# fzi-forschungszentrum-informatik/muvo

Measured on AMD Instinct MI355X. Metric: world-model training samples/sec (seq_len=10), higher is better.
Workload: dtype f32 storage/accumulate; large contractions (convolutions, transformer Linear) as bf16x3 split products

## Files before the change

### include/muvo_hip.h

```cpp
#ifndef MUVO_HIP_H
#define MUVO_HIP_H
#include <stdint.h>

#ifdef __cplusplus
extern "C" {
#endif

#define MUVO_OK 0
#define MUVO_ERR_INVALID_ARG (-1)
#define MUVO_ERR_HIP (-2)

#define MUVO_ACT_NONE 0
#define MUVO_ACT_RELU 1
#define MUVO_ACT_LEAKY 2
#define MUVO_ACT_ELU 3
#define MUVO_ACT_TANH 4
#define MUVO_ACT_SIGMOID 5

const char* muvo_last_error(void);
int muvo_abi_version(void);
int muvo_selftest_mfma(void* stream);
int muvo_set_deterministic(int on);
int muvo_reset_accumulators(void);
int muvo_get_deterministic(void);
// ... 5 lines not shown
  int32_t in_sz[3], out_sz[3];
  int32_t ksz[3], stride[3], pad[3], dil[3];
} muvo_conv_desc;

#define MUVO_CONV_F32 0
#define MUVO_CONV_BF16X3 1
#define MUVO_CONV_MODE_DEFAULT MUVO_CONV_BF16X3
int muvo_conv_set_products(int n);
int muvo_conv_get_products(void);
int muvo_conv_set_mode(int mode);
int muvo_conv_get_mode(void);
int muvo_conv_set_bf16x3_min_gflop(double gflop_per_item);
int muvo_linear_bf16x3_pack_floats(int in_f, int out_f, int64_t* fwd_floats, int64_t* dgrad_floats);
int muvo_linear_bf16x3_pack(int in_f, int out_f, const float* w, float* wp_fwd, float* wp_dgrad, void* stream);
int64_t muvo_linear_bf16x3_workspace_bytes(int64_t rows, int features);
int muvo_linear_bf16x3_split(const float* x, int64_t rows, int features, void* ws, void* stream);
int muvo_linear_bf16x3_forward(int64_t rows, int in_f, int out_f, const void* ws_x, const float* wp_fwd, const float* bias,
                               float* y, int act, float slope, void* stream);
int muvo_linear_bf16x3_dgrad(int64_t rows, int in_f, int out_f, const void* ws_dz, const float* wp_dgrad, float* dx,
                             void* stream);
int muvo_linear_bf16x3_wgrad(int64_t rows, int in_f, int out_f, const void* ws_x, const void* ws_dz, float* scratch,
                             float* dw, void* stream);
int64_t muvo_pack_table_item_bytes(void);
int muvo_conv_pack_table_add(void* host_items, int capacity, int* n_items, int64_t* n_blocks, const muvo_conv_desc* d,
                             const float* w, float* wp_fwd, float* wp_dgrad);
int muvo_linear_bf16x3_pack_table_add(void* host_items, int capacity, int* n_items, int64_t* n_blocks, int in_f, int out_f,
                                      const float* w, float* wp_fwd, float* wp_dgrad);
int muvo_pack_table_run(const void* dev_items, int n_items, int64_t n_blocks, void* stream);
int muvo_conv_pack_sizes(const muvo_conv_desc* d, int64_t* fwd_floats, int64_t* dgrad_floats);
int muvo_conv_pack_weights(const muvo_conv_desc* d, const float* w, float* wp_fwd, float* wp_dgrad, void* stream);
int64_t muvo_conv_workspace_bytes(const muvo_conv_desc* d, int op);
int muvo_conv_kernel_family(const muvo_conv_desc* d, int op);
int muvo_conv_kernel_variant(const muvo_conv_desc* d, int op);
int muvo_conv_forward(const muvo_conv_desc* d, const float* x, const float* wp_fwd, const float* bias, float* y, int act,
                      float slope, void* ws, void* stream);
int muvo_conv_dgrad(const muvo_conv_desc* d, const float* dy, const float* wp_dgrad, float* dx, void* ws, int ws_valid,
                    void* stream);
int muvo_conv_forward_head_supported(const muvo_conv_desc* d, int CO);
int muvo_conv_forward_head(const muvo_conv_desc* d, const float* x, const float* wp_fwd, const float* bias, float* y, int act,
                           float slope, void* ws, const float* head_w, const float* head_b, int CO, float* logits, void* stream);
int muvo_conv_forward_moments_supported(const muvo_conv_desc* d);
int muvo_conv_forward_moments(const muvo_conv_desc* d, const float* x, const float* wp_fwd, const float* bias, float* y, int act,
                              float slope, double* moments, void* stream);
int muvo_adain_fwd_moments(const float* x, const float* style, float* y, float* save_mean, float* save_rstd, double* moments,
                           int N, int C, int64_t S, float eps, void* stream);
int muvo_adain_affine(const float* style, double* moments, float* save_mean, float* save_rstd, float* aff, int N, int C, int64_t S,
                      float eps, void* stream);
int muvo_conv_affine_supported(const muvo_conv_desc* d);
int muvo_conv_forward_affine(const muvo_conv_desc* d, const float* x, const float* aff, const float* wp_fwd, const float* bias,
                             float* y, int act, float slope, double* moments, void* stream);
int muvo_conv_wgrad_affine(const muvo_conv_desc* d, const float* x, const float* aff, const float* dy, float* dw, float* dbias,
                           void* stream);
int muvo_grouped_linear_fwd(const float* x, int M, int K, int L, const float* const* W, const float* const* b, float* const* Y,
                            const int* N, void* stream);
int muvo_grouped_linear_bwd(const float* x, int M, int K, int L, const float* const* W, float* const* dY, float* dx,
                            float* const* dW, float* const* db, const int* N, void* stream);
int muvo_bf3_loop_clock(double* shader_mhz, double* us_per_k_step);
int muvo_adain_head_supported(int C, int CO, int64_t S);
int muvo_adain_head_fwd(const float* x, const float* style, float* save_mean, float* save_rstd, double* moments, const float* head_w,
                        const float* head_b, float* logits, int N, int C, int CO, int64_t S, float eps, void* stream);
int muvo_adain_head_bwd(const float* x, const float* style, const float* save_mean, const float* save_rstd, const float* head_w,
                        const float* dlogits, float* dx, float* dstyle, float* dhead_w, float* dhead_b, double* ws, int N, int C,
                        int CO, int64_t S, int act, float slope, void* stream);
int muvo_conv_dgrad_accumulate(const muvo_conv_desc* d, const float* dy, const float* wp_dgrad, float* dx, void* stream);
int muvo_conv_prepare_dy(const muvo_conv_desc* d, const float* y, const float* dy, int act, float slope, void* ws_dy,
                         float* dbias, void* stream);
// ... 210 lines not shown
```

### muvo_amd/csrc/conv_bf3.h

```cpp
#pragma once
#include "conv_plan.h"

void bf3_finish_phase(ConvPhase& g);
int bf3_pack_phase(const ConvPhase& g, const float* w, float* wp, hipStream_t st);
long bf3_workspace_bytes(int N, int C, long S);
int bf3_split_input(const float* x, void* ws, int N, int C, long S, hipStream_t st, const float* yact = nullptr, int act = 0,
                    float slope = 0.f, float* dbias = nullptr, const float* dhead = nullptr, const float* head_w = nullptr, int CO = 0,
                    float* dhead_w = nullptr, float* dhead_b = nullptr);
int bf3_launch_fwd_phase(const ConvPhase& g, const void* ws, const float* wp, const float* bias, float* out, int act,
                         float slope, hipStream_t st, int ksplit = 1);
void bf3_set_fused_head(const float* w, const float* b, float* out, int co);
void bf3_set_products(int n);
int bf3_get_products();
int bf3_fwd_ksplit(const ConvPhase& g);
int bf3_wgrad_phase(const ConvPhase& g, const void* ws_x, int Cin_total, const void* ws_dz, int Cout_total, float* wg,
                    float* dw, hipStream_t st);
int bf3_split_rows(const float* x, void* ws, long rows, int C, hipStream_t st);
bool bf3_fwd_uses_pp(const ConvPhase& g);
bool bf3_wgrad_uses_pp(const ConvPhase& g);
struct PackItem {
  ConvPhase g;
  const float* w;
  float* dst;
  long blk0;
  int nblk, pad_;
};
int pack_table_launch(const PackItem* dev_items, int n, long n_blocks, hipStream_t st);
```

### muvo_amd/csrc/conv_bf3.hip

```cpp
#include "conv_bf3.h"
#include <type_traits>

typedef __bf16 bf16x8 __attribute__((ext_vector_type(8)));
typedef __bf16 bf16x2 __attribute__((ext_vector_type(2)));
typedef float f32x2 __attribute__((ext_vector_type(2)));

__device__ unsigned long long g_bf3_clock[3];
extern "C" int muvo_bf3_loop_clock(double* shader_mhz, double* us_per_k_step) {
  unsigned long long h[3] = {0, 0, 0};
  if (hipMemcpyFromSymbol(h, HIP_SYMBOL(g_bf3_clock), sizeof(h)) != hipSuccess) return MUVO_ERR_HIP;
  if (h[1] == 0 || h[2] == 0) { *shader_mhz = 0.0; *us_per_k_step = 0.0; return MUVO_OK; }
  *shader_mhz = (double)h[0] / ((double)h[1] / 100.0);
  *us_per_k_step = (double)h[1] / 100.0 / (double)h[2];
  return MUVO_OK;
}

#ifdef MUVO_BF3_STAMPS
__device__ unsigned long long g_bf3_stamps[8 * 16384];
#define BF3_STAMP(slot)                                                                      \
  if (MUVO_BF3_STAMPS != 3 && threadIdx.x == 0 && blockIdx.x < 16384) g_bf3_stamps[blockIdx.x * 8 + (slot)] = __builtin_amdgcn_s_memrealtime()
extern "C" int muvo_debug_bf3_stamps_reset() {
  void* p = nullptr;
  return hipGetSymbolAddress(&p, HIP_SYMBOL(g_bf3_stamps)) == hipSuccess && hipMemset(p, 0, sizeof(unsigned long long) * 8 * 16384) == hipSuccess ? 0 : 1;
}
extern "C" int muvo_debug_bf3_stamps(unsigned long long* host_out, int n_u64) {
  return hipMemcpyFromSymbol(host_out, HIP_SYMBOL(g_bf3_stamps), sizeof(unsigned long long) * n_u64) == hipSuccess ? 0 : 1;
}
#define BF3_LINEAR_BLOCK ((blockIdx.z * gridDim.y + blockIdx.y) * gridDim.x + blockIdx.x)
#define BF3_STAMP3(slot)                                                                     \
  if (threadIdx.x == 0 && BF3_LINEAR_BLOCK < 16384) g_bf3_stamps[BF3_LINEAR_BLOCK * 8 + (slot)] = __builtin_amdgcn_s_memrealtime()
#else
#define BF3_STAMP(slot)
#define BF3_STAMP3(slot)
#endif

__device__ __forceinline__ void split2(float x0, float x1, unsigned& hi, unsigned& lo) {
  const bf16x2 h = __builtin_convertvector((f32x2){x0, x1}, bf16x2);
  hi = __builtin_bit_cast(unsigned, h);
  const float h0 = __uint_as_float(hi << 16), h1 = __uint_as_float(hi & 0xffff0000u);
  const bf16x2 l = __builtin_convertvector((f32x2){x0 - h0, x1 - h1}, bf16x2);
  lo = __builtin_bit_cast(unsigned, l);
}


typedef const __attribute__((address_space(1))) void* gptr_t;
typedef __attribute__((address_space(3))) void* lptr_t;
__host__ __device__ static inline bool bf3_tap_inner(const ConvPhase& g) { return (g.Cp & 31) == 0 && g.T > 1; }

__device__ __forceinline__ void dma16(const uint4* g, uint4* lds_wave_base) {
  __builtin_amdgcn_global_load_lds((gptr_t)g, (lptr_t)lds_wave_base, 16, 0, 0);
}

template <int BM, int BN, int WM, int WN, int BKC, int NST, bool ONE = false>
__global__ void __launch_bounds__(64 * WM * WN)
conv_bf3_kernel(const ConvPhase g, const uint4* __restrict__ xs, long plane_u4, const uint4* __restrict__ wp,
                const float* __restrict__ bias, float* __restrict__ out, int act, float slope,
                const uint4* __restrict__ zero16, int ksplit, const float* __restrict__ head_w, const float* __restrict__ head_b,
                float* __restrict__ head_out, int head_co) {
  constexpr int BK = 8 * BKC, NW = WM * WN;
  constexpr int TM = BM / (WM * 32), TN = BN / (WN * 32);
  constexpr int STAGE = 2 * BKC * (BM + BN);
  constexpr int RG = BM / 64, NG = BN / 64;
  constexpr int APW = 2 * BKC * RG / NW;
  constexpr int CPW = 2 * BKC * NG / NW;
  static_assert(APW * NW == 2 * BKC * RG && CPW * NW == 2 * BKC * NG && NW % NG == 0, "DMA roles must tile");
  constexpr int DMA_PER_STEP = APW + CPW;
  extern __shared__ uint4 smem[];
  const int tid = threadIdx.x, lane = tid & 63;
  const int wave = __builtin_amdgcn_readfirstlane(tid >> 6);
  const int wm = wave / WN, wn = wave % WN;
  BF3_STAMP(0);
#if defined(MUVO_BF3_STAMPS) && MUVO_BF3_STAMPS != 3
  if (threadIdx.x == 0 && blockIdx.x < 16384)
    g_bf3_stamps[blockIdx.x * 8 + 5] = ((unsigned long long)__builtin_amdgcn_s_getreg(63508) << 32) | __builtin_amdgcn_s_getreg(63492);
#endif

  const int gx = (g.npix + BN - 1) / BN;
  const int wg = xcd_swizzle(blockIdx.x, gridDim.x);
  const int bx = wg % gx, by = wg / gx;

  constexpr int NPS = CPW / 2;
  static_assert(CPW % 2 == 0 && NPS * NW * 16 == BN, "B load roles must tile");
  const int cp8 = g.Cp >> 3;
  int* taptab = (int*)(smem + NST * STAGE);
  for (int tt = tid; tt < g.T; tt += 64 * NW) {
    const int d = g.tap_d[tt];
    taptab[tt] = (((((d >> 16) & 255) - 128) * g.IH + ((d >> 8) & 255) - 128) * g.IW + (d & 255) - 128) * cp8;
    taptab[64 + tt] = d;
  }
  float* head_lds = (float*)(taptab + 128) + NW * (32 * TM);
  if (head_co > 0)
    for (int i = tid; i < head_co * g.Msub; i += 64 * NW) head_lds[i] = head_w[i];
  __syncthreads();
  int pixoff[NPS];
  unsigned long long vmask[NPS];
  int z0[NPS], y0[NPS], x0[NPS];
  bool pvalid[NPS];
#pragma unroll
  for (int sidx = 0; sidx < NPS; ++sidx) {
    const int p = bx * BN + (wave * NPS + sidx) * 16 + (lane >> 2);
    pvalid[sidx] = p < g.npix;
    int n, iz, iy, ix;
    decode_pix(g, pvalid[sidx] ? p : 0, n, iz, iy, ix);
    z0[sidx] = iz * g.is[0] + g.ib[0]; y0[sidx] = iy * g.is[1] + g.ib[1]; x0[sidx] = ix * g.is[2] + g.ib[2];
    pixoff[sidx] = (((n * g.ID + z0[sidx]) * g.IH + y0[sidx]) * g.IW + x0[sidx]) * cp8;
    vmask[sidx] = 0ull;
  }
#pragma unroll 3
  for (int tt = 0; tt < g.T; ++tt) {
    const int d = taptab[64 + tt];
    const int dz = ((d >> 16) & 255) - 128, dy = ((d >> 8) & 255) - 128, dx = (d & 255) - 128;
#pragma unroll
    for (int sidx = 0; sidx < NPS; ++sidx) {
      const bool ok = pvalid[sidx] && (unsigned)(z0[sidx] + dz) < (unsigned)g.ID && (unsigned)(y0[sidx] + dy) < (unsigned)g.IH &&
                      (unsigned)(x0[sidx] + dx) < (unsigned)g.IW;
      vmask[sidx] |= (unsigned long long)ok << tt;
    }
  }
  const int zero_off = (int)(2 * plane_u4);
  const int m_tile = by * BM;
  const uint4* wpb = wp + g.wp_off / 4 + m_tile;
  const int nk = g.Kp / BK;
  const int sps = (nk + ksplit - 1) / ksplit;
  const int kt0 = blockIdx.y * sps, kt1 = kt0 + sps < nk ? kt0 + sps : nk;
  if (kt0 >= kt1) return;

  float* sbias = (float*)(taptab + 128) + wave * (32 * TM);
  typedef unsigned u32x4 __attribute__((ext_vector_type(4)));
  const __amdgpu_buffer_rsrc_t rs_w = __builtin_amdgcn_make_buffer_rsrc(
      (void*)wpb, 0, (int)(((long)(g.Kp >> 5) * 8 * g.Mp - m_tile) * 16), 0x00020000);
  const __amdgpu_buffer_rsrc_t rs_x = __builtin_amdgcn_make_buffer_rsrc((void*)xs, 0, (int)(2 * plane_u4 * 16), 0x00020000);
  constexpr int OOB = 0x7ffffff0;
  u32x4 R[2][DMA_PER_STEP];
  int b_uoff = 0; unsigned long long b_bit = 0ull; bool b_tval = false;
  const bool tap_inner = bf3_tap_inner(g);
  int ti_t = kt0 % g.T, ti_c8 = (lane & 3) + 4 * (kt0 / g.T);
  auto bstate = [&](int kt) {
    if (tap_inner) {
      b_uoff = taptab[ti_t] + ti_c8;
      b_bit = 1ull << ti_t;
      b_tval = ti_c8 < cp8;
      if (++ti_t == g.T) { ti_t = 0; ti_c8 += 4; }
      return;
    }
    const int k0 = kt * BK + (lane & 3) * 8;
    const int t = (int)(((unsigned long long)(unsigned)k0 * g.cp_magic) >> 32);
    const int c8 = (k0 - t * g.Cp) >> 3;
    const int tc = t < g.T ? t : 0;
    b_uoff = taptab[tc] + c8;
    b_bit = 1ull << tc;
    b_tval = t < g.T;
  };
  auto gload_piece = [&](auto par, int kt, int q) {
    constexpr int P = decltype(par)::value;
    if (q < APW) {
      const int k32 = (kt * BK) >> 5, c4 = ((kt * BK) >> 3) & 3;
      const int a = wave * APW + q;
      const int pc = a / RG, rg = a % RG;
      const int plane = pc / BKC, ch = pc % BKC;
      R[P][q] = __builtin_bit_cast(u32x4, __builtin_amdgcn_raw_buffer_load_b128(rs_w, (ONE && plane == 1) ? OOB : lane * 16, ((k32 * 8 + plane * 4 + c4 + ch) * g.Mp + rg * 64) * 16, 0));
    } else {
      const int plane = (q - APW) & 1, sidx = (q - APW) >> 1;
      const bool ok = b_tval && (vmask[sidx] & b_bit) && !(ONE && plane == 1);
      const int off = ok ? (pixoff[sidx] + b_uoff + plane * (int)plane_u4) * 16 : OOB;
      R[P][q] = __builtin_bit_cast(u32x4, __builtin_amdgcn_raw_buffer_load_b128(rs_x, off, 0, 0));
    }
  };
  auto lstore_piece = [&](auto par, int stage, int q) {
    constexpr int P = decltype(par)::value;
    uint4* S = smem + stage * STAGE;
    if (q < APW) {
      const int a = wave * APW + q;
      const int pc = a / RG, rg = a % RG;
      *(u32x4*)(S + pc * BM + rg * 64 + lane) = R[P][q];
    } else {
      const int pl = (wave * NPS + ((q - APW) >> 1)) * 16 + (lane >> 2);
      *(u32x4*)(S + 2 * BKC * BM + ((q - APW) & 1) * BKC * BN + pl * 4 + ((lane & 3) ^ ((lane >> 4) & 3))) = R[P][q];
    }
  };

  f32x16 acc[TM][TN];
#pragma unroll
  for (int i = 0; i < TM; ++i)
#pragma unroll
    for (int j = 0; j < TN; ++j)
#pragma unroll
      for (int r = 0; r < 16; ++r) acc[i][j][r] = 0.f;

  static_assert(BKC == 4 && (NST == 2 || NST == 3), "two k-slices per step; two LDS stages, or three for the ping-pong schedule");
  const int fragA = wm * (TM * 32) + (lane & 31);
  const int fragB = 2 * BKC * BM + (wn * (TN * 32) + (lane & 31)) * 4 + ((lane >> 5) ^ ((lane >> 2) & 3));
  auto load_frags = [&](int stage, int ks, bf16x8 (&ah)[TM], bf16x8 (&al)[TM], bf16x8 (&bh)[TN], bf16x8 (&bl)[TN]) {
    const uint4* S = smem + stage * STAGE;
// ... 123 lines not shown
      __builtin_amdgcn_sched_barrier(0);
  #pragma unroll
      for (int i = 0; i < TM; ++i)
  #pragma unroll
        for (int j = 0; j < TN; ++j) {
          if constexpr (!ONE) {
            acc[i][j] = __builtin_amdgcn_mfma_f32_32x32x16_bf16(a1l[i], b1h[j], acc[i][j], 0, 0, 0);
            acc[i][j] = __builtin_amdgcn_mfma_f32_32x32x16_bf16(a1h[i], b1l[j], acc[i][j], 0, 0, 0);
          }
          acc[i][j] = __builtin_amdgcn_mfma_f32_32x32x16_bf16(a1h[i], b1h[j], acc[i][j], 0, 0, 0);
  #pragma unroll
          for (int u = 0; u < PPP; ++u)
            if ((i * TN + j) * PPP + u < DMA_PER_STEP) lstore_piece(par, P, (i * TN + j) * PPP + u);
          __builtin_amdgcn_sched_barrier(0);
        }
      __builtin_amdgcn_s_waitcnt(0xC07F);
    };
    for (int kt = kt0; kt < kt1; kt += 2) {
      step(par0{}, kt);
      if (kt + 1 < kt1) step(par1{}, kt + 1);
    }
  }

  BF3_STAMP(3);
  if (NST == 3 && blockIdx.x == 0 && threadIdx.x == 0 && gridDim.x >= 2048) {
    g_bf3_clock[0] = __builtin_amdgcn_s_memtime() - clk0;
    g_bf3_clock[1] = __builtin_amdgcn_s_memrealtime() - rt0;
    g_bf3_clock[2] = (unsigned long long)nk;
  }
#if defined(MUVO_BF3_STAMPS) && MUVO_BF3_STAMPS != 3
  if (threadIdx.x == 0 && blockIdx.x < 16384) g_bf3_stamps[blockIdx.x * 8 + 7] = __builtin_amdgcn_s_memtime() - clk0;
#endif
#define BF3_STORE(ACT) conv_tile_store<ACT, true, true>(g, acc, bias, out, slope, bx * BN, m_tile, wm, wn, lane, sbias, head_lds, head_co, head_b, head_out)
  if (ksplit > 1) conv_tile_atomic<true>(g, acc, out, bx * BN, m_tile, wm, wn, lane);
  else { MUVO_ACT_SWITCH(act, BF3_STORE) }
  BF3_STAMP(4);
#if defined(MUVO_BF3_STAMPS) && MUVO_BF3_STAMPS == 2
  __builtin_amdgcn_s_waitcnt(0);
  BF3_STAMP(6);
#endif
}

typedef short s16x4 __attribute__((ext_vector_type(4)));
typedef __attribute__((address_space(3))) s16x4* lds_s16x4_ptr;
__device__ __forceinline__ bf16x8 tr_read8(const char* lds_addr0, const char* lds_addr1) {
  const s16x4 a = __builtin_amdgcn_ds_read_tr16_b64_v4i16((lds_s16x4_ptr)lds_addr0);
  const s16x4 b = __builtin_amdgcn_ds_read_tr16_b64_v4i16((lds_s16x4_ptr)lds_addr1);
  typedef short s16x8 __attribute__((ext_vector_type(8)));
  const s16x8 v = __builtin_shufflevector(a, b, 0, 1, 2, 3, 4, 5, 6, 7);
  return __builtin_bit_cast(bf16x8, v);
}

struct WgradBlock { int x, y, z; };
__device__ __forceinline__ WgradBlock wgrad_block(int xcd_order) {
  WgradBlock b = {(int)blockIdx.x, (int)blockIdx.y, (int)blockIdx.z};
  if (xcd_order) {
    const int gx = gridDim.x, gy = gridDim.y;
    const int v = xcd_swizzle((b.z * gy + b.y) * gx + b.x, gx * gy * (int)gridDim.z);
    b.x = v % gx;
    const int r = v / gx;
    b.y = r % gy;
    b.z = r / gy;
  }
  return b;
}

template <int BM, int BN, int WM, int WN, int WK, bool ONE = false>
__global__ void __launch_bounds__(64 * WM * WN * WK)
// ... 898 lines not shown
  return MUVO_OK;
}

__global__ void __launch_bounds__(256) rows_split_kernel(const float* __restrict__ in, uint4* __restrict__ out_hi,
                                                         uint4* __restrict__ out_lo, long n_u4) {
  for (long i = blockIdx.x * 256L + threadIdx.x; i < n_u4; i += (long)gridDim.x * 256) {
    const float4 a = reinterpret_cast<const float4*>(in)[2 * i], b = reinterpret_cast<const float4*>(in)[2 * i + 1];
    uint4 h, l;
    split2(a.x, a.y, h.x, l.x);
    split2(a.z, a.w, h.y, l.y);
    split2(b.x, b.y, h.z, l.z);
    split2(b.z, b.w, h.w, l.w);
    out_hi[i] = h;
    out_lo[i] = l;
  }
  if (blockIdx.x == 0 && threadIdx.x == 0) out_hi[2 * n_u4] = make_uint4(0u, 0u, 0u, 0u);
}

int bf3_split_rows(const float* x, void* ws, long rows, int C, hipStream_t st) {
  const long n_u4 = rows * C / 8;
  uint4* hi = (uint4*)ws;
  hipLaunchKernelGGL(rows_split_kernel, dim3(ew_grid(n_u4)), dim3(256), 0, st, x, hi, hi + n_u4, n_u4);
  MUVO_CHECK_LAUNCH("rows_split_kernel");
  return MUVO_OK;
}

struct Bf3Head { const float* w; const float* b; float* out; int co; };
static thread_local Bf3Head t_bf3_head = {nullptr, nullptr, nullptr, 0};

static int g_bf3_products = 3;
void bf3_set_products(int n) { g_bf3_products = n == 1 ? 1 : 3; }
int bf3_get_products() { return g_bf3_products; }

template <int BM, int BN, int WM, int WN, int BKC, int NST, bool ONE>
static int bf3_launch_t(const ConvPhase& g, const void* ws, const float* wp, const float* bias, float* out, int act,
                        float slope, hipStream_t st, int ksplit) {
  constexpr size_t lds0 = (size_t)NST * 2 * BKC * (BM + BN) * 16 + 512 + 4 * BM * WN;
  static_assert(lds0 <= 160 * 1024, "LDS budget");
  constexpr size_t HEAD_LDS = NST == 3 ? 4096 : 0;
  const Bf3Head hd = (NST == 3 && ksplit <= 1) ? t_bf3_head : Bf3Head{nullptr, nullptr, nullptr, 0};
  const size_t lds = lds0 + (hd.co > 0 ? HEAD_LDS : 0);
  static_assert(lds0 + HEAD_LDS <= 160 * 1024, "LDS budget with a fused head");
  static bool attr_set = false;
  static const uint4* zero16 = nullptr;
  if (!attr_set) {
    if (hipFuncSetAttribute((const void*)conv_bf3_kernel<BM, BN, WM, WN, BKC, NST, ONE>, hipFuncAttributeMaxDynamicSharedMemorySize,
                            (int)(lds0 + HEAD_LDS)) != hipSuccess ||
        hipGetSymbolAddress((void**)&zero16, HIP_SYMBOL(g_zero16)) != hipSuccess) {
      muvo_set_error("conv_bf3: kernel attribute / symbol setup failed");
      return MUVO_ERR_HIP;
    }
    attr_set = true;
  }
  const long plane_u4 = (long)g.N * g.ID * g.IH * g.IW * (g.Cp / 8);
  dim3 grid(cdiv(g.npix, BN) * cdiv(g.M, BM), ksplit, 1);
  hipLaunchKernelGGL((conv_bf3_kernel<BM, BN, WM, WN, BKC, NST, ONE>), grid, dim3(64 * WM * WN), lds, st, g, (const uint4*)ws, plane_u4,
                     (const uint4*)wp, bias, out, act, slope, zero16, ksplit, hd.w, hd.b, hd.out, hd.co);
  MUVO_CHECK_LAUNCH("conv_bf3_kernel");
  return MUVO_OK;
}
template <int BM, int BN, int WM, int WN, int BKC, int NST>
static int bf3_launch(const ConvPhase& g, const void* ws, const float* wp, const float* bias, float* out, int act,
                      float slope, hipStream_t st, int ksplit = 1) {
  return g_bf3_products == 1 ? bf3_launch_t<BM, BN, WM, WN, BKC, NST, true>(g, ws, wp, bias, out, act, slope, st, ksplit)
                             : bf3_launch_t<BM, BN, WM, WN, BKC, NST, false>(g, ws, wp, bias, out, act, slope, st, ksplit);
}

bool bf3_fwd_uses_pp(const ConvPhase& g) {
  if (g.M <= 64) return false;
  const long big = g.M > 128 ? (long)cdiv(g.npix, 128) * cdiv(g.M, 256) : (long)cdiv(g.npix, 256) * cdiv(g.M, 128);
  static const int min_blocks = getenv("MUVO_BF3_PP_MIN_BLOCKS") ? atoi(getenv("MUVO_BF3_PP_MIN_BLOCKS")) : 128;
  return big >= min_blocks;
}
bool bf3_wgrad_uses_pp(const ConvPhase& g) { return g.M > 128 || (g.M > 64 && g.C > 64); }

int bf3_fwd_ksplit(const ConvPhase& g) {
  if (g.npix <= 0 || bf3_fwd_uses_pp(g) || muvo_det()) return 1;
  static const int tgt = getenv("MUVO_BF3_KSPLIT_BLOCKS") ? atoi(getenv("MUVO_BF3_KSPLIT_BLOCKS")) : 512;
  static const int min_steps = getenv("MUVO_BF3_KSPLIT_MIN_STEPS") ? atoi(getenv("MUVO_BF3_KSPLIT_MIN_STEPS")) : 16;
  const long tiles = (long)cdiv(g.npix, 128) * cdiv(g.M, 64);
  const int nk = g.Kp / 32;
  if (tiles >= 192 || nk < 2 * min_steps) return 1;
  int ks = cdiv(tgt, tiles);
  if (ks > nk / min_steps) ks = nk / min_steps;
  return ks < 1 ? 1 : ks;
}

void bf3_set_fused_head(const float* w, const float* b, float* out, int co) { t_bf3_head = Bf3Head{w, b, out, co}; }

int bf3_launch_fwd_phase(const ConvPhase& g, const void* ws, const float* wp, const float* bias, float* out, int act,
                         float slope, hipStream_t st, int ksplit) {
  if (g.npix <= 0) return MUVO_OK;
  if (ksplit > 1) return bf3_launch<64, 128, 1, 4, 4, 2>(g, ws, wp, nullptr, out, MUVO_ACT_NONE, 0.f, st, ksplit);
  static const int variant = getenv("MUVO_BF3_VARIANT") ? atoi(getenv("MUVO_BF3_VARIANT")) : 0;
  if (variant == 2) {
    if (g.M > 128) return bf3_launch<256, 128, 4, 2, 4, 2>(g, ws, wp, bias, out, act, slope, st);
    if (g.M > 64) return bf3_launch<128, 256, 2, 4, 4, 2>(g, ws, wp, bias, out, act, slope, st);
  }
  if (bf3_fwd_uses_pp(g)) {
    if (g.M > 128) return bf3_launch<256, 128, 4, 2, 4, 3>(g, ws, wp, bias, out, act, slope, st);
    return bf3_launch<128, 256, 2, 4, 4, 3>(g, ws, wp, bias, out, act, slope, st);
  }
  return bf3_launch<64, 128, 1, 4, 4, 2>(g, ws, wp, bias, out, act, slope, st);
}

static int bf3_wgrad_ksplit(long tiles, int nsteps, int tgt, int minst, int slots) {
  if (muvo_det()) return 1;
  int ksplit = cdiv(tgt, tiles);
  if (ksplit > cdiv(nsteps, minst)) ksplit = cdiv(nsteps, minst);
  if (ksplit < 1) ksplit = 1;
  static const int quant = getenv("MUVO_BF3_WGRAD_QUANT") ? atoi(getenv("MUVO_BF3_WGRAD_QUANT")) : 1;
  if (quant && tiles * ksplit < 4L * slots) {
    const int kmax = nsteps / 12 > 1 ? nsteps / 12 : 1;
    double best = 1e30;
    for (int ks = 1; ks <= kmax && tiles * ks <= 8L * slots; ++ks) {
      const int sps = cdiv(nsteps, ks);
      if (cdiv(nsteps, sps) != ks) continue;
      const double cost = (double)cdiv(tiles * ks, slots) * (sps * 1.2 + 12.0);
      if (cost < best - 1e-9) { best = cost; ksplit = ks; }
    }
  }
  return ksplit;
}

static int bf3_wgrad_xcd_order() {
  static const int v = getenv("MUVO_BF3_WGRAD_XCD") ? atoi(getenv("MUVO_BF3_WGRAD_XCD")) : 1;
  return v;
}

template <int BM, int BN, int WM, int WN, bool ONE>
static int bf3_wgrad_pp_launch_t(const ConvPhase& g, const void* ws_x, int Cin_total, const void* ws_dz, int Cout_total,
                                 float* wg, hipStream_t st) {
  constexpr size_t lds = (size_t)3 * 2 * 32 * (BM / 8 + BN / 8) * 16;
  static bool attr_set = false;
  if (!attr_set) {
    if (hipFuncSetAttribute((const void*)conv_bf3_wgrad_pp_kernel<BM, BN, WM, WN, ONE>, hipFuncAttributeMaxDynamicSharedMemorySize,
// ... 105 lines not shown
```

### muvo_amd/csrc/conv_gemm.hip

```cpp
#include "common.h"
#include "conv_vox.h"
#include "conv_pw.h"
#include "conv_plan.h"
#include "conv_bf3.h"

typedef __bf16 wg_bf16x8 __attribute__((ext_vector_type(8)));
__device__ __forceinline__ void wg_split8(const float (&v)[8], wg_bf16x8& hi, wg_bf16x8& lo) {
  typedef __bf16 b2 __attribute__((ext_vector_type(2)));
  typedef float f2 __attribute__((ext_vector_type(2)));
  unsigned h[4], l[4];
#pragma unroll
  for (int p = 0; p < 4; ++p) {
    const b2 hh = __builtin_convertvector((f2){v[2 * p], v[2 * p + 1]}, b2);
    h[p] = __builtin_bit_cast(unsigned, hh);
    const float h0 = __uint_as_float(h[p] << 16), h1 = __uint_as_float(h[p] & 0xffff0000u);
    const b2 ll = __builtin_convertvector((f2){v[2 * p] - h0, v[2 * p + 1] - h1}, b2);
    l[p] = __builtin_bit_cast(unsigned, ll);
  }
  typedef unsigned u4 __attribute__((ext_vector_type(4)));
  hi = __builtin_bit_cast(wg_bf16x8, (u4){h[0], h[1], h[2], h[3]});
  lo = __builtin_bit_cast(wg_bf16x8, (u4){l[0], l[1], l[2], l[3]});
}

template <int BM, int BN, int WM, int WN, int RUN>
// ... 692 lines not shown
                  2e-9 * (double)g.M * (double)g.npix * (double)g.T * (double)g.C >= f32_bf3_min_gflop();
  if (b3) {
    if (bn == 128) hipLaunchKernelGGL((conv_wgrad_kernel<128, 128, 2, 2, true>), grid, dim3(256), 0, st, g, in, dout, dwp, tps);
    else if (bn == 64) hipLaunchKernelGGL((conv_wgrad_kernel<128, 64, 2, 2, true>), grid, dim3(256), 0, st, g, in, dout, dwp, tps);
    else hipLaunchKernelGGL((conv_wgrad_kernel<128, 32, 4, 1, true>), grid, dim3(256), 0, st, g, in, dout, dwp, tps);
  } else {
    if (bn == 128) hipLaunchKernelGGL((conv_wgrad_kernel<128, 128, 2, 2, false>), grid, dim3(256), 0, st, g, in, dout, dwp, tps);
    else if (bn == 64) hipLaunchKernelGGL((conv_wgrad_kernel<128, 64, 2, 2, false>), grid, dim3(256), 0, st, g, in, dout, dwp, tps);
    else hipLaunchKernelGGL((conv_wgrad_kernel<128, 32, 4, 1, false>), grid, dim3(256), 0, st, g, in, dout, dwp, tps);
  }
  MUVO_CHECK_LAUNCH("conv_wgrad_kernel");
  return MUVO_OK;
}

extern "C" {

int muvo_conv_set_mode(int mode) {
  MUVO_CHECK_ARG(mode == MUVO_CONV_F32 || mode == MUVO_CONV_BF16X3, "conv_set_mode: unknown mode %d", mode);
  g_conv_mode = mode;
  return MUVO_OK;
}
int muvo_conv_get_mode(void) { return conv_mode(); }
int muvo_conv_set_products(int n) {
  MUVO_CHECK_ARG(n == 1 || n == 3, "conv_set_products: 1 (bf16) or 3 (bf16x3), got %d", n);
  bf3_set_products(n);
  return MUVO_OK;
}
int muvo_conv_get_products(void) { return bf3_get_products(); }
int muvo_conv_set_bf16x3_min_gflop(double gflop_per_item) {
  g_bf3_min_gflop = gflop_per_item < 0.0 ? -1.0 : gflop_per_item;
  return MUVO_OK;
}

int muvo_conv_pack_sizes(const muvo_conv_desc* d, int64_t* fwd_floats, int64_t* dgrad_floats) {
  ConvPlan pl;
  int rc = build_plan(d, &pl);
  if (rc) return rc;
  {
    ConvPlan pf;
    rc = build_plan(d, &pf, 0, false);
    if (rc) return rc;
    if (pf.fwd_floats > pl.fwd_floats) pl.fwd_floats = pf.fwd_floats;
  }
  if (vox_fwd_ok(d) && vox_pack_floats(d) > pl.fwd_floats) pl.fwd_floats = vox_pack_floats(d);
  if (vox_dgrad_ok(d) && vox_pack_floats(d) > pl.dgr_floats) pl.dgr_floats = vox_pack_floats(d);
  if (fwd_floats) *fwd_floats = pl.fwd_floats;
  if (dgrad_floats) *dgrad_floats = pl.dgr_floats;
  return MUVO_OK;
}

int muvo_conv_pack_weights(const muvo_conv_desc* d, const float* w, float* wp_fwd, float* wp_dgrad, void* stream) {
  ConvPlan pl;
  int rc = build_plan(d, &pl);
  if (rc) return rc;
  MUVO_CHECK_ARG(w != nullptr, "conv_pack_weights: w is null");
  hipStream_t st = (hipStream_t)stream;
  if (pw_applicable(d)) {
    const size_t bytes = sizeof(float) * d->Cout * d->Cin;
    if ((wp_fwd && hipMemcpyAsync(wp_fwd, w, bytes, hipMemcpyDeviceToDevice, st) != hipSuccess) ||
        (wp_dgrad && hipMemcpyAsync(wp_dgrad, w, bytes, hipMemcpyDeviceToDevice, st) != hipSuccess)) {
      muvo_set_error("conv_pack_weights: copy failed");
      return MUVO_ERR_HIP;
    }
    return MUVO_OK;
  }
  if (wp_fwd && vox_fwd_ok(d)) {
// ... 504 lines not shown
```

### muvo_amd/csrc/conv_plan.h

```cpp
#pragma once
#include "common.h"

#define MAX_TAPS 64

struct ConvPhase {
  int N, C, Cp, M, Mp, T, Kp;
  int ID, IH, IW;
  int OD, OH, OW;
  int SD, SH, SW;
  int os[3], op[3];
  int is[3], ib[3];
  int in_sC, out_sC;
  long in_sN, out_sN;
  int npix;
  unsigned cp_magic;
  int tap_d[MAX_TAPS];
  int tap_w[MAX_TAPS];
  long wp_off;
  long wsm, wsc;
  int bf3;
  int nmerge, Msub;
  int mop[8][3];
  int tap_wm[8][MAX_TAPS];
};
// ... 147 lines not shown
      const int mo = mb - grp * g.Msub;
      int mz = mopv[0][0], my = mopv[0][1], mx = mopv[0][2];
#pragma unroll
      for (int q = 1; q < NG; ++q) { mz = grp == q ? mopv[q][0] : mz; my = grp == q ? mopv[q][1] : my; mx = grp == q ? mopv[q][2] : mx; }
      const size_t obase = (size_t)nn * g.out_sN + ((size_t)(jz * g.os[0] + mz) * g.OH + (jy * g.os[1] + my)) * g.OW + (jx * g.os[2] + mx);
      if (VEC4 && g.out_sC == 1) {
#pragma unroll
        for (int q = 0; q < 4; ++q) {
          const int m = mo + 8 * q + 4 * (lane >> 5);
          if (m < g.M) {
            float4 v = make_float4(acc[i][j][4 * q], acc[i][j][4 * q + 1], acc[i][j][4 * q + 2], acc[i][j][4 * q + 3]);
            if (use_bias) {
              const float4 b4 = *reinterpret_cast<const float4*>(sb + i * 32 + 8 * q + 4 * (lane >> 5));
              v.x += b4.x; v.y += b4.y; v.z += b4.z; v.w += b4.w;
            }
            v.x = act_apply_c<ACT>(v.x, slope); v.y = act_apply_c<ACT>(v.y, slope);
            v.z = act_apply_c<ACT>(v.z, slope); v.w = act_apply_c<ACT>(v.w, slope);
            *reinterpret_cast<float4*>(out + obase + m) = v;
          }
        }
        continue;
      }
#pragma unroll
      for (int r = 0; r < 16; ++r) {
        const int rr = (r & 3) + 8 * (r >> 2) + 4 * (lane >> 5);
        const int m = mo + rr;
        if (mb + rr < g.M && m < g.Msub)
          out[obase + (size_t)m * g.out_sC] = act_apply_c<ACT>(acc[i][j][r] + (use_bias ? sb[i * 32 + rr] : 0.f), slope);
      }
      __builtin_amdgcn_sched_barrier(0);
    }
  }
}
```

### muvo_amd/ops.py

```python
import collections
import contextlib
import ctypes as C
import math
import os
import threading
import weakref

import torch

_HERE = os.path.dirname(os.path.abspath(__file__))
_LIB_PATH = os.environ.get('MUVO_HIP_LIB') or os.path.join(_HERE, 'libmuvo_hip.so')
_lib = None
_lock = threading.Lock()

ACT_NONE, ACT_RELU, ACT_LEAKY, ACT_ELU, ACT_TANH, ACT_SIGMOID = 0, 1, 2, 3, 4, 5


class ConvDesc(C.Structure):
    _fields_ = [('nd', C.c_int32), ('transposed', C.c_int32), ('N', C.c_int32), ('Cin', C.c_int32), ('Cout', C.c_int32),
                ('in_sz', C.c_int32 * 3), ('out_sz', C.c_int32 * 3), ('ksz', C.c_int32 * 3), ('stride', C.c_int32 * 3),
                ('pad', C.c_int32 * 3), ('dil', C.c_int32 * 3)]


class GemmDesc(C.Structure):
    _fields_ = [('M', C.c_int32), ('N', C.c_int32), ('K', C.c_int32),
                ('sam', C.c_int64), ('sak', C.c_int64), ('sbk', C.c_int64), ('sbn', C.c_int64), ('scm', C.c_int64),
                ('B1', C.c_int32), ('B2', C.c_int32),
                ('a_b1', C.c_int64), ('a_b2', C.c_int64), ('b_b1', C.c_int64), ('b_b2', C.c_int64),
                ('c_b1', C.c_int64), ('c_b2', C.c_int64),
                ('alpha', C.c_float), ('bias_div', C.c_int32), ('act', C.c_int32), ('slope', C.c_float),
                ('mode', C.c_int32)]


EXPORTS = [
    'muvo_last_error', 'muvo_abi_version', 'muvo_selftest_mfma', 'muvo_set_deterministic', 'muvo_get_deterministic', 'muvo_reset_accumulators',
    'muvo_conv_set_products', 'muvo_conv_get_products',
    'muvo_conv_set_mode', 'muvo_conv_get_mode', 'muvo_conv_set_bf16x3_min_gflop', 'muvo_conv_pack_sizes', 'muvo_conv_workspace_bytes', 'muvo_conv_kernel_family', 'muvo_conv_kernel_variant', 'muvo_conv_pack_weights', 'muvo_conv_forward', 'muvo_conv_dgrad', 'muvo_conv_prepare_dy', 'muvo_conv_wgrad', 'muvo_bias_grad_nchw',
    'muvo_gemm',
    'muvo_pack_table_item_bytes', 'muvo_conv_pack_table_add', 'muvo_linear_bf16x3_pack_table_add', 'muvo_pack_table_run',
    'muvo_linear_bf16x3_pack_floats', 'muvo_linear_bf16x3_pack', 'muvo_linear_bf16x3_workspace_bytes', 'muvo_linear_bf16x3_split',
    'muvo_linear_bf16x3_forward', 'muvo_linear_bf16x3_dgrad', 'muvo_linear_bf16x3_wgrad',
    'muvo_bn_train_fwd', 'muvo_bn_train_bwd', 'muvo_adain_fwd', 'muvo_adain_bwd',
    'muvo_add_dropout_layernorm_fwd', 'muvo_add_dropout_layernorm_bwd',
    'muvo_act_fwd', 'muvo_act_bwd', 'muvo_dropout', 'muvo_axpby', 'muvo_copy2d', 'muvo_colsum_acc', 'muvo_batchsum',
    'muvo_nchw_to_tokens', 'muvo_tokens_to_nchw', 'muvo_maxpool2d_fwd', 'muvo_maxpool2d_bwd', 'muvo_avgpool_fwd',
    'muvo_avgpool_bwd', 'muvo_upsample3d_x2_fwd', 'muvo_upsample3d_x2_bwd', 'muvo_preprocess_image',
    'muvo_preprocess_route', 'muvo_divide_scalar', 'muvo_resize_bilinear', 'muvo_resize_nearest_f32',
    'muvo_resize_nearest_u8', 'muvo_softmax_dropout_fwd', 'muvo_softmax_dropout_bwd', 'muvo_gru_fwd', 'muvo_gru_bwd',
    'muvo_rssm_sample_fwd', 'muvo_rssm_sample_bwd',
    'muvo_spatial_loss_fwd', 'muvo_spatial_loss_bwd', 'muvo_spatial_loss_masked_fwd', 'muvo_spatial_loss_masked_bwd', 'muvo_voxel_loss_stats_doubles', 'muvo_voxel_loss_coef_floats',
    'muvo_voxel_loss_fwd', 'muvo_voxel_loss_bwd', 'muvo_l1_rows_fwd', 'muvo_l1_rows_bwd', 'muvo_kl_loss_fwd',
    'muvo_kl_loss_bwd', 'muvo_adamw_step',
    'muvo_ssim_frames', 'muvo_sqdiff_frames', 'muvo_chamfer_sums', 'muvo_ssc_counts',
    'muvo_frustum_cells', 'muvo_frustum_pool_fwd', 'muvo_frustum_pool_bwd', 'muvo_depth_expectation',
    'muvo_resize_bilinear_bwd', 'muvo_softmax_channel_fwd', 'muvo_softmax_channel_bwd',
    'muvo_range_projection', 'muvo_voxel_grid', 'muvo_seg_ce_fwd', 'muvo_seg_ce_bwd', 'muvo_ssim_maps', 'muvo_ssim_bwd',
    'muvo_instance_labels', 'muvo_pixel_augment', 'muvo_preprocess_route_aug',
    'muvo_split_planes_bytes', 'muvo_split_planes', 'muvo_attention_supported', 'muvo_attention_fwd', 'muvo_attention_bwd',
    'muvo_conv_dgrad_accumulate', 'muvo_conv_forward_moments_supported', 'muvo_conv_forward_moments', 'muvo_adain_fwd_moments',
    'muvo_adain_head_supported', 'muvo_adain_head_fwd', 'muvo_adain_head_bwd', 'muvo_bf3_loop_clock',
    'muvo_grouped_linear_fwd', 'muvo_grouped_linear_bwd', 'muvo_conv_prepare_dy_head', 'muvo_conv_prepare_dy_head_supported',
    'muvo_conv_forward_head_supported', 'muvo_conv_forward_head',
    'muvo_adain_affine', 'muvo_conv_affine_supported', 'muvo_conv_forward_affine', 'muvo_conv_wgrad_affine',
    'muvo_fake_allreduce', 'muvo_resize_bilinear_aa', 'muvo_bn_train_fwd_planes', 'muvo_bn_train_bwd_planes', 'muvo_conv_forward_planes',
    'muvo_stem_conv_supported', 'muvo_stem_conv_forward', 'muvo_stem_conv_wgrad',
    'muvo_rssm_supported', 'muvo_rssm_transposed_floats', 'muvo_rssm_scratch_floats', 'muvo_rssm_forward', 'muvo_rssm_backward',
    'muvo_voxelize_scratch_bytes', 'muvo_voxelize_frames',
    'muvo_birdview_decode_frames', 'muvo_label_components_frames', 'muvo_depth_semantic_decode_frames',
    'muvo_range_projection_frames', 'muvo_voxel_grid_frames',
]
# ... 2462 lines not shown
```

Before: 26.05.

## Stage conv bf16x3 epilogue through LDS for wide 128-bit output stores

Adds a wide-store epilogue for the bf16x3 conv kernel. The output tile is staged in the now-idle pipeline LDS, then written with 128-bit buffer stores along contiguous pixels, instead of the per-lane scattered stores used before. For transposed/merged phases with stride-2 width it also remaps M rows so the two parity sub-phases sit in one tile, which lets their outputs be interleaved into contiguous 16-byte writes. The aim is to cut uncoalesced global write traffic, at the cost of extra LDS round trips, barriers and more complex indexing. It is on by default when the eligibility checks pass and can be disabled with an environment variable.

```diff
diff --git a/include/muvo_hip.h b/include/muvo_hip.h
--- a/include/muvo_hip.h
+++ b/include/muvo_hip.h
@@ -61,6 +61,7 @@
 int64_t muvo_conv_workspace_bytes(const muvo_conv_desc* d, int op);
 int muvo_conv_kernel_family(const muvo_conv_desc* d, int op);
 int muvo_conv_kernel_variant(const muvo_conv_desc* d, int op);
+int muvo_conv_store_mode(const muvo_conv_desc* d, int op);
 int muvo_conv_forward(const muvo_conv_desc* d, const float* x, const float* wp_fwd, const float* bias, float* y, int act,
                       float slope, void* ws, void* stream);
 int muvo_conv_dgrad(const muvo_conv_desc* d, const float* dy, const float* wp_dgrad, float* dx, void* ws, int ws_valid,
diff --git a/muvo_amd/csrc/conv_bf3.h b/muvo_amd/csrc/conv_bf3.h
--- a/muvo_amd/csrc/conv_bf3.h
+++ b/muvo_amd/csrc/conv_bf3.h
@@ -18,6 +18,7 @@
 int bf3_split_rows(const float* x, void* ws, long rows, int C, hipStream_t st);
 bool bf3_fwd_uses_pp(const ConvPhase& g);
 bool bf3_wgrad_uses_pp(const ConvPhase& g);
+int bf3_fwd_store_mode(const ConvPhase& g);
 struct PackItem {
   ConvPhase g;
   const float* w;
diff --git a/muvo_amd/csrc/conv_bf3.hip b/muvo_amd/csrc/conv_bf3.hip
--- a/muvo_amd/csrc/conv_bf3.hip
+++ b/muvo_amd/csrc/conv_bf3.hip
@@ -56,7 +56,7 @@
 conv_bf3_kernel(const ConvPhase g, const uint4* __restrict__ xs, long plane_u4, const uint4* __restrict__ wp,
                 const float* __restrict__ bias, float* __restrict__ out, int act, float slope,
                 const uint4* __restrict__ zero16, int ksplit, const float* __restrict__ head_w, const float* __restrict__ head_b,
-                float* __restrict__ head_out, int head_co) {
+                float* __restrict__ head_out, int head_co, int wmode) {
   constexpr int BK = 8 * BKC, NW = WM * WN;
   constexpr int TM = BM / (WM * 32), TN = BN / (WN * 32);
   constexpr int STAGE = 2 * BKC * (BM + BN);
@@ -119,7 +119,13 @@
   }
   const int zero_off = (int)(2 * plane_u4);
   const int m_tile = by * BM;
-  const uint4* wpb = wp + g.wp_off / 4 + m_tile;
+  int mrow0 = m_tile, mrow1 = m_tile + BM / 2;
+  if ((wmode >> 2) & 1) {
+    const int cpp = g.Msub / (BM / 2), pair = by / cpp;
+    mrow0 = 2 * pair * g.Msub + (by - pair * cpp) * (BM / 2);
+    mrow1 = mrow0 + g.Msub;
+  }
+  const uint4* wpb = wp + g.wp_off / 4;
   const int nk = g.Kp / BK;
   const int sps = (nk + ksplit - 1) / ksplit;
   const int kt0 = blockIdx.y * sps, kt1 = kt0 + sps < nk ? kt0 + sps : nk;
@@ -128,7 +134,7 @@
   float* sbias = (float*)(taptab + 128) + wave * (32 * TM);
   typedef unsigned u32x4 __attribute__((ext_vector_type(4)));
   const __amdgpu_buffer_rsrc_t rs_w = __builtin_amdgcn_make_buffer_rsrc(
-      (void*)wpb, 0, (int)(((long)(g.Kp >> 5) * 8 * g.Mp - m_tile) * 16), 0x00020000);
+      (void*)wpb, 0, (int)((long)(g.Kp >> 5) * 8 * g.Mp * 16), 0x00020000);
   const __amdgpu_buffer_rsrc_t rs_x = __builtin_amdgcn_make_buffer_rsrc((void*)xs, 0, (int)(2 * plane_u4 * 16), 0x00020000);
   constexpr int OOB = 0x7ffffff0;
   u32x4 R[2][DMA_PER_STEP];
@@ -158,7 +164,8 @@
       const int a = wave * APW + q;
       const int pc = a / RG, rg = a % RG;
       const int plane = pc / BKC, ch = pc % BKC;
-      R[P][q] = __builtin_bit_cast(u32x4, __builtin_amdgcn_raw_buffer_load_b128(rs_w, (ONE && plane == 1) ? OOB : lane * 16, ((k32 * 8 + plane * 4 + c4 + ch) * g.Mp + rg * 64) * 16, 0));
+      const int arow = (rg * 64 < BM / 2 ? mrow0 : mrow1) + (rg * 64) % (BM / 2);
+      R[P][q] = __builtin_bit_cast(u32x4, __builtin_amdgcn_raw_buffer_load_b128(rs_w, (ONE && plane == 1) ? OOB : lane * 16, ((k32 * 8 + plane * 4 + c4 + ch) * g.Mp + arow) * 16, 0));
     } else {
       const int plane = (q - APW) & 1, sidx = (q - APW) >> 1;
       const bool ok = b_tval && (vmask[sidx] & b_bit) && !(ONE && plane == 1);
@@ -348,8 +355,15 @@
   if (threadIdx.x == 0 && blockIdx.x < 16384) g_bf3_stamps[blockIdx.x * 8 + 7] = __builtin_amdgcn_s_memtime() - clk0;
 #endif
 #define BF3_STORE(ACT) conv_tile_store<ACT, true, true>(g, acc, bias, out, slope, bx * BN, m_tile, wm, wn, lane, sbias, head_lds, head_co, head_b, head_out)
+  constexpr bool WIDE_OK = (size_t)BM * (BN + 8) * 4 <= (size_t)NST * STAGE * 16;
+  static_assert(TM * 32 <= BM / 2 || BM == 64, "a wave's rows lie in one half of a mapped tile");
+  const int wrow = wm * (TM * 32);
+  const int m_tile_w = ((wmode >> 2) & 1) ? (wrow < BM / 2 ? mrow0 : mrow1) + (wrow & (BM / 2 - 1)) - wrow : m_tile;
+#define BF3_STORE_WIDE(ACT) conv_tile_store_wide<ACT, BM, BN, 64 * NW, TM, TN>(g, acc, bias, out, slope, bx * BN, m_tile_w, mrow0, mrow1, wm, wn, lane, tid, sbias, (float*)smem, wmode & 3, (wmode >> 4) & 15, (wmode >> 8) & 15, head_lds, head_co, head_b, head_out)
   if (ksplit > 1) conv_tile_atomic<true>(g, acc, out, bx * BN, m_tile, wm, wn, lane);
-  else { MUVO_ACT_SWITCH(act, BF3_STORE) }
+  else if (WIDE_OK && (wmode & 3)) {
+    if constexpr (WIDE_OK) { MUVO_ACT_SWITCH(act, BF3_STORE_WIDE) }
+  } else { MUVO_ACT_SWITCH(act, BF3_STORE) }
   BF3_STAMP(4);
 #if defined(MUVO_BF3_STAMPS) && MUVO_BF3_STAMPS == 2
   __builtin_amdgcn_s_waitcnt(0);
@@ -1314,6 +1328,34 @@
 void bf3_set_products(int n) { g_bf3_products = n == 1 ? 1 : 3; }
 int bf3_get_products() { return g_bf3_products; }
 
+static int ilog2_exact(int v) {
+  int l = 0;
+  while ((1 << l) < v) ++l;
+  return (1 << l) == v ? l : -1;
+}
+static int bf3_wide_mode(const ConvPhase& g, const float* out, int BM, int BN, int ksplit) {
+  const char* e = getenv("MUVO_CONV_WIDE_STORE");
+  if ((e && atoi(e) == 0) || ksplit > 1) return 0;
+  const long total_bytes = (long)g.N * g.out_sN * 4;
+  if (g.out_sC == 1 || total_bytes >= 0x7fffff00L) return 0;
+  if (((uintptr_t)out & 15) || g.out_sC % 4 || g.out_sN % 4) return 0;
+  if (g.nmerge <= 1) {
+    if (g.os[2] != 1) return 0;
+    if (g.SW % 4 == 0 && g.OW % 4 == 0 && g.mop[0][2] % 4 == 0) return 1;
+    const bool planes = g.os[0] == 1 && g.os[1] == 1 && g.mop[0][0] == 0 && g.mop[0][1] == 0 && g.mop[0][2] == 0 &&
+                        g.SD == g.OD && g.SH == g.OH && g.SW == g.OW && ((long)g.SD * g.SH * g.SW) % 4 == 0;
+    return planes ? 1 : 0;
+  }
+  if ((g.nmerge & 1) || g.os[2] != 2 || g.SW % 2 || g.OW % 4 || g.OW < 2 * g.SW) return 0;
+  for (int q = 0; q < g.nmerge; q += 2)
+    if (g.mop[q][2] != 0 || g.mop[q + 1][2] != 1 || g.mop[q + 1][0] != g.mop[q][0] || g.mop[q + 1][1] != g.mop[q][1]) return 0;
+  const int ml = ilog2_exact(g.Msub);
+  if (ml < 5 || ml > 15) return 0;
+  if (2 * g.Msub <= BM) return 2 | ml << 4 | ml << 8;
+  if (BM / 2 >= 64 && g.Msub % (BM / 2) == 0) return 2 | 4 | ilog2_exact(BM / 2) << 4 | ml << 8;
+  return 0;
+}
+
 template <int BM, int BN, int WM, int WN, int BKC, int NST, bool ONE>
 static int bf3_launch_t(const ConvPhase& g, const void* ws, const float* wp, const float* bias, float* out, int act,
                         float slope, hipStream_t st, int ksplit) {
@@ -1336,8 +1378,10 @@
   }
   const long plane_u4 = (long)g.N * g.ID * g.IH * g.IW * (g.Cp / 8);
   dim3 grid(cdiv(g.npix, BN) * cdiv(g.M, BM), ksplit, 1);
+  constexpr bool wide_ok = (size_t)BM * (BN + 8) * 4 <= (size_t)NST * 2 * BKC * (BM + BN) * 16;
+  const int wmode = wide_ok ? bf3_wide_mode(g, out, BM, BN, ksplit) : 0;
   hipLaunchKernelGGL((conv_bf3_kernel<BM, BN, WM, WN, BKC, NST, ONE>), grid, dim3(64 * WM * WN), lds, st, g, (const uint4*)ws, plane_u4,
-                     (const uint4*)wp, bias, out, act, slope, zero16, ksplit, hd.w, hd.b, hd.out, hd.co);
+                     (const uint4*)wp, bias, out, act, slope, zero16, ksplit, hd.w, hd.b, hd.out, hd.co, wmode);
   MUVO_CHECK_LAUNCH("conv_bf3_kernel");
   return MUVO_OK;
 }
@@ -1351,8 +1395,8 @@
 bool bf3_fwd_uses_pp(const ConvPhase& g) {
   if (g.M <= 64) return false;
   const long big = g.M > 128 ? (long)cdiv(g.npix, 128) * cdiv(g.M, 256) : (long)cdiv(g.npix, 256) * cdiv(g.M, 128);
-  static const int min_blocks = getenv("MUVO_BF3_PP_MIN_BLOCKS") ? atoi(getenv("MUVO_BF3_PP_MIN_BLOCKS")) : 128;
-  return big >= min_blocks;
+  const char* e = getenv("MUVO_BF3_PP_MIN_BLOCKS");
+  return big >= (e ? atoi(e) : 128);
 }
 bool bf3_wgrad_uses_pp(const ConvPhase& g) { return g.M > 128 || (g.M > 64 && g.C > 64); }
 
@@ -1384,6 +1428,14 @@
     return bf3_launch<128, 256, 2, 4, 4, 3>(g, ws, wp, bias, out, act, slope, st);
   }
   return bf3_launch<64, 128, 1, 4, 4, 2>(g, ws, wp, bias, out, act, slope, st);
+}
+
+int bf3_fwd_store_mode(const ConvPhase& g) {
+  if (g.npix <= 0 || bf3_fwd_ksplit(g) > 1) return 0;
+  const bool pp = bf3_fwd_uses_pp(g);
+  if (pp && getenv("MUVO_BF3_VARIANT") && atoi(getenv("MUVO_BF3_VARIANT")) == 2) return 0;
+  const int BM = !pp ? 64 : g.M > 128 ? 256 : 128, BN = !pp ? 128 : g.M > 128 ? 128 : 256;
+  return bf3_wide_mode(g, nullptr, BM, BN, 1) & 7;
 }
 
 static int bf3_wgrad_ksplit(long tiles, int nsteps, int tgt, int minst, int slots) {
diff --git a/muvo_amd/csrc/conv_gemm.hip b/muvo_amd/csrc/conv_gemm.hip
--- a/muvo_amd/csrc/conv_gemm.hip
+++ b/muvo_amd/csrc/conv_gemm.hip
@@ -748,6 +748,15 @@
   return MUVO_OK;
 }
 
+int muvo_conv_store_mode(const muvo_conv_desc* d, int op) {
+  if ((op != 0 && op != 1) || muvo_conv_kernel_family(d, op) != 1) return 0;
+  ConvPlan pl;
+  if (build_plan(d, &pl)) return 0;
+  const ConvPhase* ph = op == 0 ? pl.fwd : pl.dgr;
+  const int nph = op == 0 ? pl.nfwd : pl.ndgr;
+  return nph > 0 ? bf3_fwd_store_mode(ph[0]) : 0;
+}
+
 int muvo_conv_pack_sizes(const muvo_conv_desc* d, int64_t* fwd_floats, int64_t* dgrad_floats) {
   ConvPlan pl;
   int rc = build_plan(d, &pl);
diff --git a/muvo_amd/csrc/conv_plan.h b/muvo_amd/csrc/conv_plan.h
--- a/muvo_amd/csrc/conv_plan.h
+++ b/muvo_amd/csrc/conv_plan.h
@@ -203,3 +203,144 @@
     }
   }
 }
+
+template <int ACT, int BM, int BN, int NT, int TM, int TN, class V>
+__device__ __forceinline__ void conv_tile_store_wide(const ConvPhase& g, const V (&acc)[TM][TN], const float* __restrict__ bias,
+                                                     float* __restrict__ out, float slope, int pix0, int m_tile_w, int mrow0,
+                                                     int mrow1, int wm, int wn, int lane, int tid, float* sb, float* stage,
+                                                     int mode, int hs_log2, int msub_log2, const float* hw, int hco,
+                                                     const float* __restrict__ hb, float* __restrict__ hlogits) {
+  constexpr int LS = BN + 8;
+  int mopv[8][3];
+#pragma unroll
+  for (int q = 0; q < 8; ++q)
+#pragma unroll
+    for (int k = 0; k < 3; ++k) mopv[q][k] = __builtin_amdgcn_readfirstlane(g.mop[q][k]);
+  const bool use_bias = bias != nullptr;
+  if (use_bias) {
+    if (lane < 32 * TM) {
+      const int mb = m_tile_w + wm * (TM * 32) + (lane & ~31);
+      const int mo = mb - (g.nmerge > 1 ? mb / g.Msub : 0) * g.Msub;
+      const int rr = lane & 31;
+      sb[lane] = (mb + rr < g.M && mo + rr < g.Msub) ? bias[mo + rr] : 0.f;
+    }
+    __builtin_amdgcn_sched_barrier(0);
+  }
+  __syncthreads();
+  const int r0 = 4 * (lane >> 5);
+#pragma unroll
+  for (int j = 0; j < TN; ++j) {
+    const int pl = wn * (TN * 32) + j * 32 + (lane & 31);
+    float hacc[4] = {0.f, 0.f, 0.f, 0.f};
+#pragma unroll
+    for (int i = 0; i < TM; ++i) {
+      const int mb = m_tile_w + wm * (TM * 32) + i * 32;
+      const int mo = mb - (g.nmerge > 1 ? mb / g.Msub : 0) * g.Msub;
+      float* trow = stage + (wm * (TM * 32) + i * 32 + r0) * LS + pl;
+#pragma unroll
+      for (int q = 0; q < 4; ++q) {
+        float b4[4] = {0.f, 0.f, 0.f, 0.f};
+        if (use_bias) {
+          const float4 t = *reinterpret_cast<const float4*>(sb + i * 32 + 8 * q + r0);
+          b4[0] = t.x; b4[1] = t.y; b4[2] = t.z; b4[3] = t.w;
+        }
+        float vq[4];
+#pragma unroll
+        for (int e = 0; e < 4; ++e) {
+          vq[e] = act_apply_c<ACT>(acc[i][j][4 * q + e] + b4[e], slope);
+          trow[(8 * q + e) * LS] = vq[e];
+        }
+        if (hco > 0) {
+#pragma unroll
+          for (int k = 0; k < 4; ++k)
+            if (k < hco) {
+              const float4 w4 = *reinterpret_cast<const float4*>(hw + k * g.Msub + mo + 8 * q + r0);
+              hacc[k] += (w4.x * vq[0] + w4.y * vq[1]) + (w4.z * vq[2] + w4.w * vq[3]);
+            }
+        }
+      }
+      __builtin_amdgcn_sched_barrier(0);
+    }
+    if (hco > 0) {
+      const int pj = pix0 + pl;
+      const bool pix_ok = pj < g.npix;
+      int nn, jz, jy, jx;
+      decode_pix(g, pix_ok ? pj : 0, nn, jz, jy, jx);
+      const int mb0 = m_tile_w + wm * (TM * 32);
+      const int grp = g.nmerge > 1 ? mb0 / g.Msub : 0;
+      const int mo0 = mb0 - grp * g.Msub;
+      int mz = mopv[0][0], my = mopv[0][1], mx = mopv[0][2];
+#pragma unroll
+      for (int q = 1; q < 8; ++q) { mz = grp == q ? mopv[q][0] : mz; my = grp == q ? mopv[q][1] : my; mx = grp == q ? mopv[q][2] : mx; }
+      const size_t hsp = ((size_t)(jz * g.os[0] + mz) * g.OH + (jy * g.os[1] + my)) * g.OW + (jx * g.os[2] + mx);
+      const bool split = g.Msub > TM * 32;
+#pragma unroll
+      for (int k = 0; k < 4; ++k)
+        if (k < hco) {
+          float h = hacc[k] + __shfl_xor(hacc[k], 32, 64);
+          if (lane < 32 && pix_ok) {
+            float* dst = hlogits + ((size_t)nn * hco + k) * g.out_sC + hsp;
+            const float bk = hb != nullptr ? hb[k] : 0.f;
+            if (split) atomicAdd(dst, h + (mo0 == 0 ? bk : 0.f));
+            else *dst = h + bk;
+          }
+        }
+    }
+  }
+  __syncthreads();
+  const long total_bytes = (long)g.N * g.out_sN * 4;
+  const __amdgpu_buffer_rsrc_t rs = __builtin_amdgcn_make_buffer_rsrc((void*)out, 0, (int)total_bytes, 0x00020000);
+  const unsigned sC4 = (unsigned)g.out_sC * 4u;
+  constexpr unsigned OOB = 0x80000000u;
+  typedef float f32x4_t __attribute__((ext_vector_type(4)));
+  typedef float f32x2_t __attribute__((ext_vector_type(2)));
+  typedef unsigned u32x4_t __attribute__((ext_vector_type(4)));
+  if (mode == 1) {
+    constexpr int PPL = BN / 4, LSTEP = NT / PPL, ITER = BM / LSTEP;
+    const int c = tid % PPL, l0 = tid / PPL;
+    const int pj = pix0 + 4 * c;
+    const bool pix_ok = pj < g.npix;
+    int nn, jz, jy, jx;
+    decode_pix(g, pix_ok ? pj : 0, nn, jz, jy, jx);
+    const size_t obase = (size_t)nn * g.out_sN + ((size_t)(jz * g.os[0] + mopv[0][0]) * g.OH + (jy * g.os[1] + mopv[0][1])) * g.OW +
+                         (jx * g.os[2] + mopv[0][2]);
+    const int m = mrow0 + l0;
+    const unsigned v0 = pix_ok ? (unsigned)(obase * 4) + (unsigned)m * sC4 : OOB;
+    const float* src = stage + l0 * LS + 4 * c;
+#pragma unroll
+    for (int it = 0; it < ITER; ++it) {
+      const f32x4_t v = *reinterpret_cast<const f32x4_t*>(src + it * LSTEP * LS);
+      const unsigned vo = m + it * LSTEP < g.M ? v0 : OOB;
+      __builtin_amdgcn_raw_buffer_store_b128(__builtin_bit_cast(u32x4_t, v), rs, vo,
+                                             (unsigned)(it * LSTEP) * sC4, 0);
+    }
+    return;
+  }
+  constexpr int PPL = BN / 2, LSTEP = NT / PPL, ITER = (BM / 2) / LSTEP;
+  const int c = tid % PPL;
+  const int l0 = __builtin_amdgcn_readfirstlane(tid / PPL);
+  const int pj = pix0 + 2 * c;
+  const bool pix_ok = pj < g.npix;
+  int nn, jz, jy, jx;
+  decode_pix(g, pix_ok ? pj : 0, nn, jz, jy, jx);
+  const size_t obase = (size_t)nn * g.out_sN + ((size_t)(jz * g.os[0]) * g.OH + jy * g.os[1]) * g.OW + jx * g.os[2];
+  const unsigned v0 = pix_ok ? (unsigned)(obase * 4) : OOB;
+  const int hs = 1 << hs_log2;
+  const unsigned ohw4 = (unsigned)g.OW * 4u;
+#pragma unroll
+  for (int it = 0; it < ITER; ++it) {
+    const int l = l0 + it * LSTEP;
+    const int ra = ((l >> hs_log2) << (hs_log2 + 1)) + (l & (hs - 1));
+    const int ma = (ra < BM / 2 ? mrow0 : mrow1) + (ra & (BM / 2 - 1));
+    if (ma >= g.M) continue;
+    const int grp = ma >> msub_log2, mo = ma & ((1 << msub_log2) - 1);
+    int mz = mopv[0][0], my = mopv[0][1];
+#pragma unroll
+    for (int q = 2; q < 8; q += 2) { mz = grp == q ? mopv[q][0] : mz; my = grp == q ? mopv[q][1] : my; }
+    const unsigned so = (unsigned)(mz * g.OH + my) * ohw4 + (unsigned)mo * sC4;
+    const f32x2_t a = *reinterpret_cast<const f32x2_t*>(stage + ra * LS + 2 * c);
+    const f32x2_t b = *reinterpret_cast<const f32x2_t*>(stage + (ra + hs) * LS + 2 * c);
+    const u32x4_t v = {__float_as_uint(a[0]), __float_as_uint(b[0]), __float_as_uint(a[1]), __float_as_uint(b[1])};
+    __builtin_amdgcn_raw_buffer_store_b128(v, rs, v0, so, 0);
+  }
+}
diff --git a/muvo_amd/ops.py b/muvo_amd/ops.py
--- a/muvo_amd/ops.py
+++ b/muvo_amd/ops.py
@@ -35,7 +35,7 @@
 EXPORTS = [
     'muvo_last_error', 'muvo_abi_version', 'muvo_selftest_mfma', 'muvo_set_deterministic', 'muvo_get_deterministic', 'muvo_reset_accumulators',
     'muvo_conv_set_products', 'muvo_conv_get_products',
-    'muvo_conv_set_mode', 'muvo_conv_get_mode', 'muvo_conv_set_bf16x3_min_gflop', 'muvo_conv_pack_sizes', 'muvo_conv_workspace_bytes', 'muvo_conv_kernel_family', 'muvo_conv_kernel_variant', 'muvo_conv_pack_weights', 'muvo_conv_forward', 'muvo_conv_dgrad', 'muvo_conv_prepare_dy', 'muvo_conv_wgrad', 'muvo_bias_grad_nchw',
+    'muvo_conv_set_mode', 'muvo_conv_get_mode', 'muvo_conv_set_bf16x3_min_gflop', 'muvo_conv_pack_sizes', 'muvo_conv_workspace_bytes', 'muvo_conv_kernel_family', 'muvo_conv_kernel_variant', 'muvo_conv_store_mode', 'muvo_conv_pack_weights', 'muvo_conv_forward', 'muvo_conv_dgrad', 'muvo_conv_prepare_dy', 'muvo_conv_wgrad', 'muvo_bias_grad_nchw',
     'muvo_gemm',
     'muvo_pack_table_item_bytes', 'muvo_conv_pack_table_add', 'muvo_linear_bf16x3_pack_table_add', 'muvo_pack_table_run',
     'muvo_linear_bf16x3_pack_floats', 'muvo_linear_bf16x3_pack', 'muvo_linear_bf16x3_workspace_bytes', 'muvo_linear_bf16x3_split',
```

After: 25.94. Within noise of the previous version (-0.4%).
